# amazon-science/instruct-video-to-video

Hardware: AMD Instinct MI355X
Metric: denoised video-frames/sec (16f@256x384, 50 DDIM steps) (higher is better)
Workload: dtype fp16; 1 GPU; C2: 1 clip/step = VAE-encode + 50 DDIM steps (3-way CFG, text 7.5 / video 1.5) + VAE-decode, 16 frames @ 256x384, random-init full-width UNet+VAE; 5 independent clips in flight per GPU (stacked into every UNet launch, B = 3 x clips); frames=16, height=256, width=384, ddim_steps=50, clips_per_gpu=5, parallelism=clip-parallel x1, one all_gather, hip_graph=True, cfg_branch_streams=False, concurrent_clips=5, clip_mode=stacked, driver_mode=False, full=False

## Files before the change

### instruct-video-to-video_amd/csrc/gemm.hip

```cpp
#include "common.h"
#include <algorithm>
#include "gemm_dma.h"
#include <type_traits>
#include <cstdlib>

typedef unsigned uint4r __attribute__((ext_vector_type(4)));

struct RowInfo {
    int base;
    int oh, ow;
    bool valid;
};

#ifdef INSV2V_GEMM_PROF
__device__ unsigned long long g_prof[8];
#define PROF_MARK(i) do { if (tid == 0) prof_t[i] = wall_clock64(); } while (0)
#else
#define PROF_MARK(i) do { } while (0)
#endif

template <int W>
__device__ __forceinline__ float lane_group_sum(float v) {
    static_assert(W == 4 || W == 8 || W == 16, "a DPP row is 16 lanes");
    auto dpp = [](float x, auto ctrl) {
// ... 910 lines not shown
        if (b11 >= 200 || nk < 64) return 1;
        s = (int)(512 / b11);
        if (s > nk / 16) s = nk / 16;
        if (s > 8) s = 8;
    }
    if (s < 2) return 1;
    if ((int64_t)s * d.M * d.N * 4 > d.workspace_bytes) return 1;
    return s;
}

static int stats_tile_width(const insv2v_gemm_desc& d) {
    if (d.mode != INSV2V_MODE_LINEAR || d.c_fp32 || d.act == INSV2V_ACT_GEGLU || d.batch > 1 || (d.N & 7) || (d.ldc & 7) ||
        ((uintptr_t)d.c & 15) || (d.residual && ((d.ldr & 7) || ((uintptr_t)d.residual & 15) || (int64_t)d.M * d.ldr * 2 >= ((int64_t)1 << 31))))
        return 0;
    int shape = d.tile % 10;
    if (d.tile >= 240 && d.tile <= 249) return (d.N % 320 || d.k_split) ? 0 : 160;
    if (d.tile >= 100) return 0;
    if (d.tile == 0) {
        insv2v_gemm_desc dd = d;
        if (!dd.stats_out) dd.stats_out = (float*)(uintptr_t)16;
        if (dd.batch <= 0) dd.batch = 1;
        if (pick_pingpong(dd) == 2) return 160;
    }
    if (shape == 0) shape = pick_tile(d);
    switch (shape) {
        case 1: case 2: case 5: case 6: case 8: return 128;
        case 3: case 4: case 7: case 9: return 64;
    }
    return 0;
}

static int64_t g_operand_window = 0;
extern "C" int64_t insv2v_set_operand_window(int64_t bytes) {
    const int64_t prev = g_operand_window;
    g_operand_window = bytes > 0 ? bytes : 0;
    return prev;
}
static int64_t operand_window() { return g_operand_window > 0 ? g_operand_window : ((int64_t)1 << 31) - ((int64_t)1 << 20); }
static bool beyond_window(const insv2v_gemm_desc& d) {
    const bool conv = d.mode == INSV2V_MODE_CONV3X3;
    const int64_t a_rows = conv ? (int64_t)d.NB * d.IH * d.IW : (int64_t)d.M;
    const int64_t esz = d.c_fp32 ? 4 : 2;
    const int64_t big_in = std::max(a_rows * d.lda * 2, d.k_split ? a_rows * d.lda2 * 2 : (int64_t)0);
    const int64_t big_out = std::max((int64_t)d.M * d.ldc * esz, d.residual ? (int64_t)d.M * d.ldr * 2 : (int64_t)0);
    return big_in >= operand_window() || big_out >= operand_window();
}

extern "C" int insv2v_gemm_stats_parts(const insv2v_gemm_desc* dp) {
    if (!dp) return 0;
    insv2v_gemm_desc d = *dp;
    if (d.batch <= 0) d.batch = 1;
    if (beyond_window(d)) return 0;
    const int w = stats_tile_width(d);
    return w ? (d.N + w - 1) / w : 0;
}

static insv2v_gemm_desc finished_stats_of(insv2v_gemm_desc dd, hipStream_t s) {
    if (dd.stats_parts > 0) {
        hipLaunchKernelGGL(ln_finalize_kernel, dim3((dd.M + 255) / 256), dim3(256), 0, s, (const float2*)dd.row_stats,
                           (float2*)dd.stats_scratch, dd.M, dd.stats_parts, dd.K, dd.ln_eps);
        dd.row_stats = dd.stats_scratch; dd.stats_parts = 0;
    }
    return dd;
}

extern "C" int insv2v_gemm(const insv2v_gemm_desc* dp, insv2v_stream_t stream) {
    if (!one_device()) return INSV2V_EINVAL;
    if (!dp) return INSV2V_EINVAL;
    insv2v_gemm_desc d = *dp;
    if (!d.a || !d.w || !d.c || d.M <= 0 || d.N <= 0 || d.K <= 0) return INSV2V_EINVAL;
    if ((d.K & 7) || (d.lda & 7) || (d.ldw & 7)) return INSV2V_EINVAL;
    if (((uintptr_t)d.a | (uintptr_t)d.w) & 15) return INSV2V_EINVAL;
    if (d.k_split) {
        if (!d.a2 || (d.k_split % BK) || (d.lda2 & 7) || ((uintptr_t)d.a2 & 15)) return INSV2V_EINVAL;
    }
    if (d.row_bias && d.rows_per_group <= 0) return INSV2V_EINVAL;
    if (d.row_stats && (!d.col_sum || d.batch > 1)) return INSV2V_EINVAL;
    if (d.stats_parts < 0 || (d.stats_parts > 0 && (!d.row_stats || !d.stats_scratch))) return INSV2V_EINVAL;
    if (d.stats_out && stats_tile_width(d) == 0) return INSV2V_EUNSUPPORTED;
    if (d.act == INSV2V_ACT_GEGLU && (d.N % 64)) return INSV2V_EINVAL;
    if (d.act < 0 || d.act > INSV2V_ACT_TANH) return INSV2V_EINVAL;
    if (d.batch <= 0) d.batch = 1;
    if (d.alpha == 0.f) d.alpha = 1.f;
    if (d.w_group_rows < 0 || (d.w_group_rows > 0 && (d.w_group_rows % 256 || d.w_group_stride <= 0))) return INSV2V_EINVAL;
    if (d.w_group_rows > 0) {
        if (d.mode != INSV2V_MODE_LINEAR || d.batch > 1 || d.c_fp32 || d.act != INSV2V_ACT_NONE || d.residual || d.row_bias || d.row_stats || d.stats_out ||
            d.k_split || d.split_k > 1 || d.K < 256 || (d.N % 256 && d.N % 320))
            return INSV2V_EUNSUPPORTED;
    }
    if (d.gn_ab && (d.mode != INSV2V_MODE_CONV3X3 || d.gn_images_per_sample <= 0 || d.upsample)) return INSV2V_EINVAL;
    if (d.mode == INSV2V_MODE_CONV3X3) {
        if (d.Cin <= 0 || (d.Cin % BK) || d.K != 9 * d.Cin) return INSV2V_EINVAL;
        if ((long)d.NB * d.OH * d.OW != d.M || d.stride < 1) return INSV2V_EINVAL;
        if (d.upsample && (d.stride != 1 || d.pad_t != 1 || d.pad_l != 1 || (d.OH != 2 * d.IH && d.OH != 2 * d.IH - 1) || (d.OW != 2 * d.IW && d.OW != 2 * d.IW - 1)))
            return INSV2V_EINVAL;
    } else if (d.mode != INSV2V_MODE_LINEAR) {
        return INSV2V_EUNSUPPORTED;
    }
    {
        const bool conv = d.mode == INSV2V_MODE_CONV3X3;
        const int64_t lim = operand_window();
        if ((int64_t)d.N * d.ldw * 2 >= ((int64_t)1 << 31)) return INSV2V_EUNSUPPORTED;
        const int64_t esz = d.c_fp32 ? 4 : 2;
        if (beyond_window(d)) {
            if (d.batch > 1 || d.stats_out || d.split_k > 1) return INSV2V_EUNSUPPORTED;
            insv2v_gemm_desc f = finished_stats_of(d, as_stream(stream));
            auto lcm = [](int64_t a, int64_t b) { int64_t x = a, y = b; while (y) { const int64_t t = x % y; x = y; y = t; } return a / x * b; };
            const int64_t opix = conv ? (int64_t)d.OH * d.OW : 1, ipix = conv ? (int64_t)d.IH * d.IW : 1;
            int64_t unit = conv ? 1 : 2;
            if (d.row_bias) {
                const int64_t grp = (int64_t)d.rows_per_group * (d.rb_mod > 0 ? d.rb_mod : 1);
                if (conv && grp % opix) return INSV2V_EUNSUPPORTED;
                unit = lcm(unit, conv ? grp / opix : grp);
            }
            if (conv && d.gn_ab) unit = lcm(unit, d.gn_images_per_sample);
            if (!conv && unit < 256) unit = lcm(unit, 256);
            if (f.w_group_rows > 0) unit = lcm(unit, f.w_group_rows);
            const int64_t total = conv ? d.NB : d.M;
            const int64_t in_row = std::max((int64_t)d.lda * 2, d.k_split ? (int64_t)d.lda2 * 2 : (int64_t)0) * ipix;
            const int64_t out_row = std::max((int64_t)d.ldc * esz, d.residual ? (int64_t)d.ldr * 2 : (int64_t)0) * opix;
            int64_t per = (lim - 1) / std::max(in_row, out_row) / unit * unit;
            if (per <= 0) return INSV2V_EUNSUPPORTED;
            const int64_t nparts = (total + per - 1) / per;
            per = ((total + nparts - 1) / nparts + unit - 1) / unit * unit;
            for (int64_t u0 = 0; u0 < total; u0 += per) {
                const int64_t nu = std::min(per, total - u0);
                insv2v_gemm_desc s = f;
                const int64_t r_in = u0 * ipix, r_out = u0 * opix;
                s.a = (const char*)f.a + r_in * f.lda * 2;
                if (f.k_split) s.a2 = (const char*)f.a2 + r_in * f.lda2 * 2;
                s.c = (char*)f.c + r_out * f.ldc * esz;
                if (f.residual) s.residual = (const char*)f.residual + r_out * f.ldr * 2;
                if (f.row_stats) s.row_stats = f.row_stats + r_out * 2;
                if (f.w_group_rows > 0) s.w = (const char*)f.w + (r_out / f.w_group_rows) * f.w_group_stride * 2;
                if (f.row_bias && f.rb_mod <= 0) s.row_bias = f.row_bias + (r_out / f.rows_per_group) * f.ld_rb;
                if (conv && f.gn_ab) s.gn_ab = f.gn_ab + (u0 / f.gn_images_per_sample) * (int64_t)f.Cin * 2;
                s.M = (int32_t)(nu * opix);
                if (conv) s.NB = (int32_t)nu;
                const int rc = insv2v_gemm(&s, stream);
                if (rc != 0) return rc;
            }
            return 0;
        }
    }
    if (d.w_group_rows > 0) {
        const int64_t groups = ((int64_t)d.M + d.w_group_rows - 1) / d.w_group_rows;
        if (groups * d.w_group_stride * 2 >= ((int64_t)1 << 31)) return INSV2V_EUNSUPPORTED;
        const int cus = num_cus_gemm();
        const long tm = (d.M + 255) / 256, q_tiles = tm * ((d.N + 255) / 256), r_tiles = tm * ((d.N + 319) / 320);
        const bool r_ok = d.N % 320 == 0, q_ok = d.N % 256 == 0;
        const double q_cost = (double)((q_tiles + cus - 1) / cus) * 256 * 1.03, r_cost = (double)((r_tiles + cus - 1) / cus) * 320;
        const bool use_r = d.tile / 10 == 24 ? true : d.tile / 10 == 23 ? false : (r_ok && (!q_ok || r_cost <= q_cost));
        if (use_r ? !r_ok : !q_ok) return INSV2V_EUNSUPPORTED;
        return use_r ? insv2v_gemm_r8(d, 0, as_stream(stream)) : insv2v_gemm_q8(d, 0, as_stream(stream));
    }
    auto finished_stats = [&](const insv2v_gemm_desc& dd) { return finished_stats_of(dd, as_stream(stream)); };
    if (d.tile >= 200 && d.tile <= 206) return INSV2V_EUNSUPPORTED;
    if (d.tile >= 230 && d.tile <= 239) {
        if (d.split_k > 1 || d.stats_out) return INSV2V_EUNSUPPORTED;
        d.split_k = 1;
        return insv2v_gemm_q8(finished_stats(d), d.tile - 230, as_stream(stream));
    }
    if (d.tile >= 240 && d.tile <= 249) {
        if (d.split_k > 1) return INSV2V_EUNSUPPORTED;
        d.split_k = 1;
        return insv2v_gemm_r8(finished_stats(d), d.tile - 240, as_stream(stream));
    }
    if (d.tile >= 210 && d.tile <= 221) {
        if (d.split_k > 1 || d.stats_out) return INSV2V_EUNSUPPORTED;
        d.split_k = 1;
        return insv2v_gemm_w4(finished_stats(d), d.tile - 210, as_stream(stream));
    }
    int shape = d.tile % 10, pipe = d.tile / 10;
    const int nsplit = d.stats_out ? 1 : pick_split(d);
    insv2v_gemm_desc full = d;
    if (nsplit > 1) {
        d.c = d.workspace; d.ldc = d.N; d.c_fp32 = 1; d.c_bs = 0;
        d.bias = nullptr; d.row_bias = nullptr; d.residual = nullptr; d.act = INSV2V_ACT_NONE; d.alpha = 1.f;
        d.row_stats = nullptr; d.col_sum = nullptr;
        d.split_k = nsplit;
        if (shape == 0) shape = 5;
    } else {
        d.split_k = 1;
    }
    if (nsplit <= 1 && d.tile == 0 && !d.gn_ab) {
        const int pp = pick_pingpong(d);
        if (pp) {
            const insv2v_gemm_desc dd = finished_stats(d);
            const int rc = pp == 2 ? insv2v_gemm_r8(dd, 0, as_stream(stream)) : insv2v_gemm_q8(dd, 0, as_stream(stream));
            if (rc != INSV2V_EUNSUPPORTED || d.stats_out) return rc;
        }
    }
    if (nsplit <= 1 && d.tile == 0 && !d.stats_out && d.act == INSV2V_ACT_GEGLU && d.mode == INSV2V_MODE_LINEAR && !d.k_split && !d.residual) {
        static const int r8_geglu = getenv("INSV2V_R8_GEGLU") ? atoi(getenv("INSV2V_R8_GEGLU")) : 1;
        const int cus = num_cus_gemm();
        if (r8_geglu && cus > 0 && d.N % 320 == 0 && d.M >= 8192 && d.K >= 640 && !d.c_fp32 && d.batch <= 1) {
            const long tm = (d.M + 255) / 256, q_tiles = tm * ((d.N + 255) / 256), r_tiles = tm * (d.N / 320);
            const double q_cost = (double)((q_tiles + cus - 1) / cus) * 256 * 1.03, r_cost = (double)((r_tiles + cus - 1) / cus) * 320;
            if (r_cost <= q_cost) {
                const int rc = insv2v_gemm_r8(finished_stats(d), 0, as_stream(stream));
                if (rc != INSV2V_EUNSUPPORTED) return rc;
            }
        }
    }
    if (nsplit <= 1 && d.tile == 0 && !d.stats_out) {
        const int pick = pick_persistent(d);
        if (pick) {
            const insv2v_gemm_desc dd = finished_stats(d);
            const int rc = pick == 1 ? insv2v_gemm_q8(dd, 0, as_stream(stream)) : insv2v_gemm_w4(dd, 0, as_stream(stream));
            if (rc != INSV2V_EUNSUPPORTED) return rc;
        }
    }
    if (nsplit <= 1 && (d.tile == 100 || d.tile == 0)) {
        const int tws = halo_tw_shift(d);
        if (d.tile == 100 && tws < 0) return INSV2V_EUNSUPPORTED;
        if (d.tile == 100 && d.act >= INSV2V_ACT_RELU) return INSV2V_EUNSUPPORTED;
        if (tws >= 0 && d.act < INSV2V_ACT_RELU && (d.tile == 100 || ((long)d.M / 128) * ((d.N + 127) / 128) >= 200))
            return d.gn_ab ? launch_halo<4, 2, 1, 2, 1, true>(d, tws, as_stream(stream)) : launch_halo<4, 2, 1, 2, 1>(d, tws, as_stream(stream));
    }
    if (d.gn_ab) return INSV2V_EUNSUPPORTED;
    if (nsplit <= 1 && d.tile == 0 && d.mode == INSV2V_MODE_CONV3X3 && d.batch == 1 && !d.c_fp32 && d.M >= 10240 && d.N >= 640 && d.K >= 5760) {
        static const int enabled = getenv("INSV2V_GEMM_PERSISTENT") ? atoi(getenv("INSV2V_GEMM_PERSISTENT")) : 1;
        if (enabled) {
            const int rc = insv2v_gemm_q8(d, 0, as_stream(stream));
            if (rc != INSV2V_EUNSUPPORTED) return rc;
        }
    }
    if (d.tile >= 101 && d.tile <= 103 && d.act >= INSV2V_ACT_RELU) return INSV2V_EUNSUPPORTED;
    if (nsplit <= 1 && d.tile == 103) {
        int tws = halo_tw_shift(d);
        if (tws < 0 || d.gn_ab) return INSV2V_EUNSUPPORTED;
        if (d.OH % 16 == 0 && d.OW % 16 == 0) tws = 4;
        else if (d.OH % 32 == 0 && d.OW % 8 == 0) tws = 3;
        else return INSV2V_EUNSUPPORTED;
        return launch_halo<8, 2, 1, 2, 1, false, 3>(d, tws, as_stream(stream));
    }
    if (nsplit <= 1 && d.tile == 102) {
        const int tws = halo_tw_shift(d);
        if (tws < 0 || d.gn_ab) return INSV2V_EUNSUPPORTED;
        return launch_halo<2, 2, 2, 2, 1>(d, tws, as_stream(stream));
    }
    if (nsplit <= 1 && d.tile == 101) {
        const int tws = halo_tw_shift(d);
        if (tws < 0) return INSV2V_EUNSUPPORTED;
        return launch_halo<2, 2, 2, 2, 2>(d, tws, as_stream(stream));
    }
    if (shape == 0) shape = pick_tile(d);
    if (d.act == INSV2V_ACT_GEGLU && (shape == 3 || shape == 4 || shape == 7 || shape == 9)) shape = 2;
    if (pipe == 0) pipe = 2;
    hipStream_t s = as_stream(stream);
    const bool conv = d.mode == INSV2V_MODE_CONV3X3;
    int rc = INSV2V_EINVAL;
    switch (pipe) {
        case 2: rc = conv ? dispatch_tile<INSV2V_MODE_CONV3X3, 2>(d, shape, s) : dispatch_tile<INSV2V_MODE_LINEAR, 2>(d, shape, s); break;
        case 3: rc = conv ? dispatch_tile<INSV2V_MODE_CONV3X3, 3>(d, shape, s) : dispatch_tile<INSV2V_MODE_LINEAR, 3>(d, shape, s); break;
        case 4: rc = conv ? dispatch_tile<INSV2V_MODE_CONV3X3, 4>(d, shape, s) : dispatch_tile<INSV2V_MODE_LINEAR, 4>(d, shape, s); break;
    }
    if (rc != 0 || nsplit <= 1) return rc;
    const int64_t nchunk = (int64_t)full.M * (full.N / 8);
    hipLaunchKernelGGL(splitk_reduce_kernel, dim3((unsigned)((nchunk + 255) / 256)), dim3(256), 0, s, full, (const float*)full.workspace, nsplit);
    return launch_status();
}

extern "C" int insv2v_conv3x3_fuses_groupnorm(const insv2v_gemm_desc* dp) {
    if (!dp || dp->mode != INSV2V_MODE_CONV3X3 || dp->upsample || dp->split_k > 1) return 0;
    insv2v_gemm_desc d = *dp;
    if (d.batch <= 0) d.batch = 1;
    if (d.tile != 0 && d.tile != 100) return 0;
    if (halo_tw_shift(d) < 0) return 0;
    if (d.tile == 0 && (pick_split(d) > 1 || ((long)d.M / 128) * ((d.N + 127) / 128) < 200)) return 0;
    return 1;
}

#ifdef INSV2V_GEMM_PROF
extern "C" int insv2v_prof_read(unsigned long long* out, int reset) {
    hipError_t e = hipMemcpyFromSymbol(out, HIP_SYMBOL(g_prof), sizeof(unsigned long long) * 8);
    if (e == hipSuccess && reset) {
        unsigned long long z[8] = {0, 0, 0, 0, 0, 0, 0, 0};
        e = hipMemcpyToSymbol(HIP_SYMBOL(g_prof), z, sizeof(z));
    }
    return (int)e;
}
#endif
```

### instruct-video-to-video_amd/csrc/gemm_r8.hip

```cpp
#include "common.h"
#include "gemm_dma.h"
#include <type_traits>
#include <cstdlib>

namespace {

constexpr int BM = 256, BN = 320;
constexpr int AH_B = 128 * 128;
constexpr int WB_B = 64 * 128;
constexpr int W_BASE = 4 * AH_B;
constexpr int RING_B = 4 * AH_B + 10 * WB_B;
constexpr int PK_BIAS = 0, PK_CS = 2048, PK_ST = 4096, PK_RB = 6144, PARK_B = 8192;
constexpr int LDS_B = RING_B + 2 * PARK_B;

#ifndef R8_MID_SPREAD
#define R8_MID_SPREAD 1
#endif
#define SB() __builtin_amdgcn_sched_barrier(0)
#define BARRIER() do { SB(); __builtin_amdgcn_s_barrier(); SB(); } while (0)

typedef unsigned uint4v __attribute__((ext_vector_type(4)));
typedef unsigned uint2v __attribute__((ext_vector_type(2)));
__device__ __forceinline__ unsigned pack_h2(float x, float y) {
    typedef float f2_t __attribute__((ext_vector_type(2)));
    const f2_t v = {x, y};
    return __builtin_bit_cast(unsigned, __builtin_convertvector(v, half2v));
}
__device__ __forceinline__ float h_lo(unsigned u) { return (float)__builtin_bit_cast(half2v, u)[0]; }
__device__ __forceinline__ float h_hi(unsigned u) { return (float)__builtin_bit_cast(half2v, u)[1]; }

template <int I> using ic = std::integral_constant<int, I>;

template <int MODE, bool HAS_RES, int DBG = 0, bool SPLIT = true, bool STATS = false, bool GEGLU = false, bool CIM = false>
__global__ __launch_bounds__(512) void gemm_r8_kernel(insv2v_gemm_desc p, int dephase) {
    extern __shared__ __attribute__((aligned(16))) char smem[];
    const int tid = threadIdx.x, lane = tid & 63;
    const int wid = __builtin_amdgcn_readfirstlane(tid >> 6);
    const int wm = wid >> 1, wn = wid & 1, grp = wid >> 2;
    const int G = (int)gridDim.x;
    constexpr bool LIN = MODE == INSV2V_MODE_LINEAR;

    const int tiles_n = (p.N + BN - 1) / BN, tiles_m = (p.M + BM - 1) / BM, ntiles = tiles_m * tiles_n;
    if (dephase > 0 && ntiles > G) {
        const int n0 = ntiles % G;
        if (n0 != 0 && (int)blockIdx.x >= n0) {
            const float tile_cycles = (float)(p.K / BK) * 3700.f + (HAS_RES ? 30000.f : 10000.f);
            const float frac = (float)((int)blockIdx.x - n0 + 1) / (float)(G - n0 + 1) * (float)dephase * 0.001f;
            const unsigned long long wait = (unsigned long long)(frac * tile_cycles);
            unsigned long long t0, t1;
            asm volatile("s_memtime %0\n\ts_waitcnt lgkmcnt(0)" : "=s"(t0)::"memory");
            do {
                __builtin_amdgcn_s_sleep(64);
                asm volatile("s_memtime %0\n\ts_waitcnt lgkmcnt(0)" : "=s"(t1)::"memory");
            } while (t1 - t0 < wait);
        }
    }
    auto tile_origin = [&](int v, int& bm0, int& bn0) {
        const int bid = xcd_remap(v, ntiles);
        constexpr int GROUP_M = 8;
        const int per_group = GROUP_M * tiles_n;
        const int gidx = bid / per_group, first_m = gidx * GROUP_M;
        const int gsz = min(GROUP_M, tiles_m - first_m), rin = bid - gidx * per_group;
        const int tn = rin / gsz, tm = first_m + rin - tn * gsz;
        bm0 = tm * BM; bn0 = tn * BN;
    };

    const srd_t rA = make_srd(p.a), rA2 = make_srd(p.a2 ? p.a2 : p.a), rW = make_srd(p.w);
    const bool ln = p.row_stats != nullptr;

    const int prow = wid * 8 + (lane >> 3);
    const int chunk8 = ((lane & 7) ^ ((prow >> 1) & 7)) * 8;
    unsigned aoff[4];
    unsigned amask[2] = {0, 0};
    unsigned woff;
    unsigned amax = 0;
    const unsigned wmax = (unsigned)(((int64_t)(p.N - 1) * p.ldw + chunk8) * 2);
    const int nk = p.K / BK;
    const int IHu = p.upsample ? p.OH : p.IH, IWu = p.upsample ? p.OW : p.IW;
    const int ups = p.upsample ? 1 : 0;
    struct Cursor { int v, kt, k0, kh, kw, ci0, soffA, abm0; bool second; int tap, dpix; unsigned wbase; } cur = {(int)blockIdx.x, 0, 0, 0, 0, 0, 0, 0, false, 0, 0, 0u};
    if (CIM) cur.dpix = -p.IW - 1;
    auto refresh_aoff = [&]() {
        const int ld = (int)((SPLIT && cur.second) ? p.lda2 : p.lda);
        if (LIN) {
            aoff[0] = ((unsigned)(cur.abm0 + prow) * (unsigned)ld + (unsigned)chunk8) * 2u;
            amax = ((unsigned)(p.M - 1) * (unsigned)ld + (unsigned)chunk8) * 2u;
        } else {
            const float rOW = 1.0f / (float)p.OW, rOH = 1.0f / (float)p.OH;
#pragma unroll
            for (int r = 0; r < 4; ++r) {
                const int m = cur.abm0 + (r >> 1) * 128 + (r & 1) * 64 + prow;
                const bool okm = m < p.M;
                const int mm = okm ? m : 0;
                int t = (int)((float)mm * rOW);
                int ow = mm - t * p.OW;
                if (ow < 0) { ow += p.OW; --t; } else if (ow >= p.OW) { ow -= p.OW; ++t; }
                int nb = (int)((float)t * rOH);
                int oh = t - nb * p.OH;
                if (oh < 0) { oh += p.OH; --nb; } else if (oh >= p.OH) { oh -= p.OH; ++nb; }
                if (CIM) {
                    aoff[r] = (unsigned)(nb * p.IH * p.IW + oh * p.IW + ow);
                    const unsigned vh = (okm && oh > 0 ? 1u : 0u) | (okm ? 2u : 0u) | (okm && oh + 1 < p.IH ? 4u : 0u);
                    const unsigned vw = (ow > 0 ? 1u : 0u) | 2u | (ow + 1 < p.IW ? 4u : 0u);
                    const unsigned bits = ((vh & 1u) ? vw : 0u) | ((vh & 2u) ? vw << 3 : 0u) | ((vh & 4u) ? vw << 6 : 0u);
                    if (r & 1) amask[r >> 1] |= bits << 9; else amask[r >> 1] = bits;
                } else {
                    const int ih = oh * p.stride - p.pad_t + cur.kh, iw = ow * p.stride - p.pad_l + cur.kw;
                    const bool ok = okm && (unsigned)ih < (unsigned)IHu && (unsigned)iw < (unsigned)IWu;
                    const int pix = nb * p.IH * p.IW + (ih >> ups) * p.IW + (iw >> ups);
                    aoff[r] = ok ? (unsigned)((pix * ld + chunk8) * 2) : OOB_OFFSET;
                }
            }
        }
    };
    auto set_stage_rows = [&](int v) {
        int bm0 = 0, bn0 = 0;
        const bool live = v < ntiles;
        if (live) tile_origin(v, bm0, bn0);
        else { bm0 = p.M + BM; bn0 = p.N + BN; }
        cur.abm0 = bm0;
        cur.wbase = (LIN && live && p.w_group_rows > 0) ? (unsigned)((int64_t)(bm0 / p.w_group_rows) * p.w_group_stride * 2) : 0u;
        const int c32 = (wid & 3) * 8 + (lane >> 3);
        const int pc = ((c32 >> 2) & 3) * 8 + (c32 >> 4) * 4 + (c32 & 3);
        const int n = GEGLU ? bn0 + (c32 >> 4) * 32 + (c32 & 15) : bn0 + (wid >> 2) * 160 + pc;
        woff = ((unsigned)n * (unsigned)p.ldw + (unsigned)chunk8) * 2u;
    };
    auto advance = [&]() {
        bool newtile = false, refresh = false;
        if (++cur.kt == nk) {
            cur.v += G; cur.kt = 0; cur.k0 = 0; cur.kh = cur.kw = cur.ci0 = 0; cur.soffA = 0; cur.second = false;
            if (CIM) { cur.tap = 0; cur.dpix = -p.IW - 1; }
            newtile = true;
        } else if (CIM) {
            if (++cur.tap == 9) { cur.tap = 0; cur.ci0 += BK; }
            const int kh = (cur.tap * 11) >> 5, kw = cur.tap - 3 * kh;
            cur.dpix = (kh - 1) * p.IW + kw - 1;
            cur.second = SPLIT && p.k_split > 0 && cur.ci0 >= p.k_split;
            cur.soffA = (cur.ci0 - (cur.second ? p.k_split : 0)) * 2;
            cur.k0 = cur.tap * p.Cin + cur.ci0;
        } else {
            cur.k0 += BK; cur.soffA += BK * 2;
            if (LIN) {
                if (SPLIT && p.k_split > 0 && cur.k0 == p.k_split) { cur.second = true; cur.soffA = 0; refresh = true; }
            } else {
                cur.ci0 += BK;
                if (cur.ci0 >= p.Cin) {
                    cur.ci0 = 0; cur.soffA = 0;
                    if (++cur.kw == 3) { cur.kw = 0; ++cur.kh; }
                    cur.second = false; refresh = true;
                } else if (SPLIT && p.k_split > 0 && cur.ci0 == p.k_split) {
                    cur.second = true; cur.soffA = 0; refresh = true;
                }
            }
        }
        if (newtile) set_stage_rows(cur.v);
        if (newtile || refresh) refresh_aoff();
    };
    auto stage_a = [&](auto h_c, auto buf_c, int i) {
        constexpr int H = decltype(h_c)::value, BUF = decltype(buf_c)::value;
        char* dst = smem + (H * 2 + BUF) * AH_B + i * 8192 + wid * 1024;
        if (LIN) {
            const int ld = (int)((SPLIT && cur.second) ? p.lda2 : p.lda);
            dma16((SPLIT && cur.second) ? rA2 : rA, min(aoff[0] + (unsigned)((H * 128 + i * 64) * ld * 2), amax), cur.soffA, dst);
        } else if (CIM) {
            constexpr int R = H * 2;
            const unsigned ld2 = (unsigned)((SPLIT && cur.second) ? p.lda2 : p.lda) * 2u;
            const bool ok = (amask[H] >> (i * 9 + cur.tap)) & 1u;
            const unsigned off = __umul24(aoff[R + i] + (unsigned)cur.dpix, ld2) + (unsigned)(chunk8 * 2);
            dma16((SPLIT && cur.second) ? rA2 : rA, ok ? off : OOB_OFFSET, cur.soffA, dst);
        } else {
            dma16((SPLIT && cur.second) ? rA2 : rA, aoff[H * 2 + i], cur.soffA, dst);
        }
    };
    auto stage_w = [&](auto pb_c, auto buf_c) {
        constexpr int PB = decltype(pb_c)::value, BUF = decltype(buf_c)::value;
        char* dst = smem + W_BASE + (PB * 2 + BUF) * WB_B + wid * 1024;
        if (GEGLU) {
            const int t = (wid >> 2) * 5 + PB;
            dma16(rW, min(woff + (unsigned)(((t >> 1) * 64 + (t & 1) * 16) * (int)p.ldw * 2), wmax), cur.k0 * 2 + (int)cur.wbase, dst);
        } else {
            dma16(rW, min(woff + (unsigned)(PB * 32 * (int)p.ldw * 2), wmax), cur.k0 * 2 + (int)cur.wbase, dst);
        }
    };
    auto row_group = [&](int m) { int g = m / p.rows_per_group; if (p.rb_mod > 0) g %= p.rb_mod; return g; };
    auto stage_park = [&](int pb, int bm0, int bn0) {
        char* park = smem + RING_B + pb * PARK_B;
        const srd_t rBias = make_srd(p.bias ? (const void*)p.bias : p.w), rCs = make_srd(ln ? (const void*)p.col_sum : p.w),
// ... 103 lines not shown
    const unsigned lds0 = (unsigned)(uintptr_t)(__attribute__((address_space(3))) char*)smem;
    auto park6 = [&](unsigned a, floatx4& b0, floatx4& b1, floatx4& r0, floatx4& r1, floatx4& c0, floatx4& c1) {
        if constexpr (GEGLU)
            asm volatile("ds_read_b128 %0, %6\n\tds_read_b128 %1, %6 offset:128\n\tds_read_b128 %2, %6 offset:6144\n\t"
                         "ds_read_b128 %3, %6 offset:6272\n\tds_read_b128 %4, %6 offset:2048\n\tds_read_b128 %5, %6 offset:2176\n\t"
                         "s_waitcnt lgkmcnt(0)"
                         : "=&v"(b0), "=&v"(b1), "=&v"(r0), "=&v"(r1), "=&v"(c0), "=&v"(c1) : "v"(a) : "memory");
        else
            asm volatile("ds_read_b128 %0, %6\n\tds_read_b128 %1, %6 offset:16\n\tds_read_b128 %2, %6 offset:6144\n\t"
                         "ds_read_b128 %3, %6 offset:6160\n\tds_read_b128 %4, %6 offset:2048\n\tds_read_b128 %5, %6 offset:2064\n\t"
                         "s_waitcnt lgkmcnt(0)"
                         : "=&v"(b0), "=&v"(b1), "=&v"(r0), "=&v"(r1), "=&v"(c0), "=&v"(c1) : "v"(a) : "memory");
    };
    auto stat4 = [&](unsigned a, float2& s0, float2& s1, float2& s2, float2& s3) {
        asm volatile("ds_read_b64 %0, %4\n\tds_read_b64 %1, %4 offset:128\n\tds_read_b64 %2, %4 offset:256\n\tds_read_b64 %3, %4 offset:384\n\t"
                     "s_waitcnt lgkmcnt(0)" : "=&v"(s0), "=&v"(s1), "=&v"(s2), "=&v"(s3) : "v"(a) : "memory");
    };
    auto epilogue = [&](int bm0, int bn0, int pb) {
        if (DBG == 2 || DBG == 5) {
            float s = 0.f;
#pragma unroll
            for (int i = 0; i < 5; ++i)
#pragma unroll
                for (int tb = 0; tb < 4; ++tb)
#pragma unroll
                    for (int cb = 0; cb < 2; ++cb)
#pragma unroll
                        for (int r = 0; r < 4; ++r) s += acc[i][tb][cb][r];
            if (s == 12345.678f) ((half_t*)p.c)[tid] = (half_t)s;
            return;
        }
        unsigned elane;
        asm volatile("v_mbcnt_lo_u32_b32 %0, -1, 0\n\tv_mbcnt_hi_u32_b32 %0, -1, %0" : "=v"(elane));
        const int e15 = (int)(elane & 15), eg = (int)(elane >> 4);
        const srd_t rC = make_srd(p.c), rR = make_srd(p.residual ? p.residual : p.c);
        const unsigned park = lds0 + RING_B + pb * PARK_B;
        float ra[LIN ? 4 : 1], rm[LIN ? 4 : 1];
        unsigned offc[4], offr[4];
        {
            float2 st[4];
            if (LIN) stat4(park + PK_ST + (wm * 64 + e15) * 8, st[0], st[1], st[2], st[3]);
            else { ra[0] = p.alpha; rm[0] = 0.f; }
#pragma unroll
            for (int tb = 0; tb < 4; ++tb) {
                const int m = bm0 + wm * 64 + tb * 16 + e15;
                if (LIN) {
                    const float mean = ln ? st[tb].x : 0.f, rstd = ln ? st[tb].y : 1.f;
                    ra[tb] = rstd * p.alpha; rm[tb] = -rstd * mean;
                }
                offc[tb] = m < p.M ? (unsigned)(m * (int)p.ldc * 2 + eg * (GEGLU ? 8 : 16)) : OOB_OFFSET;
                offr[tb] = m < p.M ? (unsigned)(m * (int)p.ldr * 2 + eg * 16) : OOB_OFFSET;
            }
        }
        if constexpr (GEGLU) {
#pragma unroll
            for (int pbk = 0; pbk < 5; ++pbk) {
                const int t = wn * 5 + pbk;
                const int nl = (t >> 1) * 64 + (t & 1) * 16 + 4 * eg;
                float bh[4], ch[4], bg[4], cg[4];
                {
                    floatx4 tb_[2], tr[2], tc[2];
                    park6(park + nl * 4, tb_[0], tb_[1], tr[0], tr[1], tc[0], tc[1]);
#pragma unroll
                    for (int e = 0; e < 4; ++e) { bh[e] = tb_[0][e] + tr[0][e]; ch[e] = tc[0][e]; bg[e] = tb_[1][e] + tr[1][e]; cg[e] = tc[1][e]; }
                }
                const int on = (bn0 >> 1) + t * 16;
                const bool okc = on + eg * 4 + 4 <= (p.N >> 1);
#pragma unroll
                for (int tb = 0; tb < 4; ++tb) {
                    float v[4];
#pragma unroll
                    for (int e = 0; e < 4; ++e) {
                        const float x = fmaf(ra[LIN ? tb : 0], acc[pbk][tb][0][e], fmaf(rm[LIN ? tb : 0], ch[e], bh[e]));
                        const float g = fmaf(ra[LIN ? tb : 0], acc[pbk][tb][1][e], fmaf(rm[LIN ? tb : 0], cg[e], bg[e]));
                        v[e] = x * gelu_erf_f(g);
                    }
                    const uint2v out = {pack_h2(v[0], v[1]), pack_h2(v[2], v[3])};
                    __builtin_amdgcn_raw_buffer_store_b64(out, rC, okc ? offc[tb] : OOB_OFFSET, on * 2, 0);
                    asm volatile("s_nop 7" ::"v"(out));
                }
            }
            return;
        }
        uint4v rv[2][4];
        auto load_res = [&](auto pbk_c, auto slot_c) {
            constexpr int PBK = decltype(pbk_c)::value, SLOT = decltype(slot_c)::value;
            const int on = bn0 + wn * 160 + PBK * 32;
            const bool okc = on + eg * 8 + 8 <= p.N;
#pragma unroll
            for (int tb = 0; tb < 4; ++tb) rv[SLOT][tb] = __builtin_amdgcn_raw_buffer_load_b128(rR, okc ? offr[tb] : OOB_OFFSET, on * 2, 0);
        };
        if (HAS_RES) {
            load_res(ic<0>{}, ic<0>{}); load_res(ic<1>{}, ic<1>{});
            asm volatile("s_waitcnt vmcnt(0)" ::: "memory");
            SB();
        }
        float st1[4] = {0.f, 0.f, 0.f, 0.f}, st2[4] = {0.f, 0.f, 0.f, 0.f};
#pragma unroll
        for (int pbk = 0; pbk < 5; ++pbk) {
            const int slot = pbk & 1;
            if (HAS_RES && (pbk == 2 || pbk == 4)) { asm volatile("s_waitcnt vmcnt(0)" ::: "memory"); SB(); }
            const int cl = wn * 160 + pbk * 32 + 8 * eg;
            float bs[8], cs[8];
            {
                floatx4 tb_[2], tr[2], tc[2];
                park6(park + cl * 4, tb_[0], tb_[1], tr[0], tr[1], tc[0], tc[1]);
#pragma unroll
                for (int h = 0; h < 2; ++h)
#pragma unroll
                    for (int e = 0; e < 4; ++e) { bs[4 * h + e] = tb_[h][e] + tr[h][e]; cs[4 * h + e] = tc[h][e]; }
            }
            const int on = bn0 + wn * 160 + pbk * 32;
            const bool okc = on + eg * 8 + 8 <= p.N;
#pragma unroll
            for (int tb = 0; tb < 4; ++tb) {
                float v[8];
#pragma unroll
                for (int h = 0; h < 2; ++h)
#pragma unroll
                    for (int e = 0; e < 4; ++e) v[4 * h + e] = fmaf(ra[LIN ? tb : 0], acc[pbk][tb][h][e], fmaf(rm[LIN ? tb : 0], cs[4 * h + e], bs[4 * h + e]));
                if (HAS_RES) {
                    const uint4v r = rv[slot][tb];
                    v[0] += h_lo(r[0]); v[1] += h_hi(r[0]); v[2] += h_lo(r[1]); v[3] += h_hi(r[1]);
                    v[4] += h_lo(r[2]); v[5] += h_hi(r[2]); v[6] += h_lo(r[3]); v[7] += h_hi(r[3]);
                }
                if (STATS) {
#pragma unroll
                    for (int e = 0; e < 8; ++e) { st1[tb] += v[e]; st2[tb] = fmaf(v[e], v[e], st2[tb]); }
                }
                const uint4v out = {pack_h2(v[0], v[1]), pack_h2(v[2], v[3]), pack_h2(v[4], v[5]), pack_h2(v[6], v[7])};
                __builtin_amdgcn_raw_buffer_store_b128(out, rC, okc ? offc[tb] : OOB_OFFSET, on * 2, 0);
                asm volatile("s_nop 7" ::"v"(out));
            }
            if (HAS_RES) {
                SB();
                if (pbk == 0) load_res(ic<2>{}, ic<0>{});
                if (pbk == 1) load_res(ic<3>{}, ic<1>{});
                if (pbk == 2) load_res(ic<4>{}, ic<0>{});
                SB();
            }
        }
        if (STATS) {
            const int part = bn0 / 160 + wn;
#pragma unroll
            for (int tb = 0; tb < 4; ++tb) {
                const int m = bm0 + wm * 64 + tb * 16 + e15;
                float s1 = st1[tb] + __shfl_xor(st1[tb], 16, 64), s2 = st2[tb] + __shfl_xor(st2[tb], 16, 64);
                s1 += __shfl_xor(s1, 32, 64); s2 += __shfl_xor(s2, 32, 64);
                if (eg == 0 && m < p.M) *(float2*)(p.stats_out + ((int64_t)part * p.M + m) * 2) = make_float2(s1, s2);
            }
        }
    };

    int cbm0, cbn0;
    int cv = blockIdx.x, cpb = 0;
    tile_origin(cv, cbm0, cbn0);
    set_stage_rows(cv);
    refresh_aoff();
    stage_park(0, cbm0, cbn0);
    stage_a(ic<0>{}, ic<0>{}, 0); stage_a(ic<0>{}, ic<0>{}, 1); stage_a(ic<1>{}, ic<0>{}, 0); stage_a(ic<1>{}, ic<0>{}, 1);
    stage_w(ic<0>{}, ic<0>{}); stage_w(ic<1>{}, ic<0>{}); stage_w(ic<2>{}, ic<0>{}); stage_w(ic<3>{}, ic<0>{}); stage_w(ic<4>{}, ic<0>{});
    advance();
    stage_a(ic<0>{}, ic<1>{}, 0); stage_a(ic<0>{}, ic<1>{}, 1); stage_a(ic<1>{}, ic<1>{}, 0); stage_a(ic<1>{}, ic<1>{}, 1);
    stage_w(ic<0>{}, ic<1>{}); stage_w(ic<1>{}, ic<1>{});
    wait_vmcnt<6>();
    BARRIER();
    zero_acc();

    auto tile_step = [&](auto buf_c, bool first, int nbm0, int nbn0, int npb) {
        constexpr int B = decltype(buf_c)::value;
        read_w(ic<B>{}, ic<0>{});
        SB();
        read_a(ic<B>{});
        SB();
        if (first) stage_park(npb, nbm0, nbn0);
        BARRIER();
        mma(ic<0>{}, [&](int i) { if (i == 0) stage_w(ic<2>{}, ic<B ^ 1>{}); else stage_w(ic<3>{}, ic<B ^ 1>{}); });
        BARRIER();
        read_w(ic<B>{}, ic<1>{});
        BARRIER();
        mma(ic<1>{}, [&](int i) { if (i == 0) stage_w(ic<4>{}, ic<B ^ 1>{}); });
        BARRIER();
        read_w(ic<B>{}, ic<2>{});
        advance();
        BARRIER();
        mma(ic<2>{}, [&](int i) { stage_a(ic<0>{}, ic<B>{}, i); });
        BARRIER();
        read_w(ic<B>{}, ic<3>{});
        BARRIER();
        mma(ic<3>{}, [&](int i) { stage_a(ic<1>{}, ic<B>{}, i); });
        BARRIER();
        read_w(ic<B>{}, ic<4>{});
        wait_vmcnt<4>();
        BARRIER();
        mma(ic<4>{}, [&](int i) { if (i == 0) stage_w(ic<0>{}, ic<B>{}); else stage_w(ic<1>{}, ic<B>{}); });
        BARRIER();
    };
    int par = 0;
    unsigned long long cyc_loop = 0, cyc_join = 0, cyc_epi = 0, ntl = 0, ts0 = 0, ts1 = 0, ts2 = 0, ts3 = 0;
    auto stamp = [&](unsigned long long& t) { if (DBG == 4) asm volatile("s_memtime %0\n\ts_waitcnt lgkmcnt(0)" : "=s"(t)::"memory"); };
    for (; cv < ntiles; cv += G) {
        tile_origin(cv, cbm0, cbn0);
        stamp(ts0);
        if (grp == 1) BARRIER();
        bool first = cv != (int)blockIdx.x;
        int t = 0;
        if (par) { tile_step(ic<1>{}, first, cbm0, cbn0, cpb); first = false; t = 1; par = 0; }
        for (; t + 1 < nk; t += 2) {
            tile_step(ic<0>{}, first, cbm0, cbn0, cpb);
            first = false;
            tile_step(ic<1>{}, false, cbm0, cbn0, cpb);
        }
        if (t < nk) { tile_step(ic<0>{}, first, cbm0, cbn0, cpb); par = 1; }
        stamp(ts1);
        if (grp == 0) BARRIER();
        stamp(ts2);
        epilogue(cbm0, cbn0, cpb);
        stamp(ts3);
        if (DBG == 4) { cyc_loop += ts1 - ts0; cyc_join += ts2 - ts1; cyc_epi += ts3 - ts2; ++ntl; }
        zero_acc();
        cpb ^= 1;
    }
    if (DBG == 5 && p.workspace && blockIdx.x < 64 && lane == 0) {
        unsigned* o = (unsigned*)p.workspace + ((int)blockIdx.x * 8 + wid) * 12;
#pragma unroll
        for (int i = 0; i < 5; ++i) { o[i] = dbg_seg[i]; o[5 + i] = dbg_gap[i]; }
        o[10] = dbg_n; o[11] = 0;
    }
    if (DBG == 4 && p.workspace && blockIdx.x < 64 && lane == 0) {
        unsigned long long* o = (unsigned long long*)p.workspace + ((int)blockIdx.x * 8 + wid) * 4;
        o[0] = cyc_loop; o[1] = cyc_join; o[2] = cyc_epi; o[3] = ntl;
    }
}

template <int MODE, bool HAS_RES, int DBG = 0, bool SPLIT = true, bool STATS = false, bool GEGLU = false, bool CIM = false>
int launch_r8(const insv2v_gemm_desc& d, hipStream_t s) {
    static bool attr_set = false;
    static int num_cu = 0;
    if (!attr_set) {
        hipError_t e = hipFuncSetAttribute((const void*)gemm_r8_kernel<MODE, HAS_RES, DBG, SPLIT, STATS, GEGLU, CIM>, hipFuncAttributeMaxDynamicSharedMemorySize, LDS_B);
        if (e != hipSuccess) return (int)e;
        int dev = 0;
        hipDeviceProp_t prop;
        if (hipGetDevice(&dev) != hipSuccess || hipGetDeviceProperties(&prop, dev) != hipSuccess) return INSV2V_EINVAL;
        num_cu = prop.multiProcessorCount;
        attr_set = true;
    }
    const int tiles = ((d.M + BM - 1) / BM) * ((d.N + BN - 1) / BN);
    static const int dephase = getenv("INSV2V_R8_DEPHASE") ? atoi(getenv("INSV2V_R8_DEPHASE")) : 0;
    hipLaunchKernelGGL((gemm_r8_kernel<MODE, HAS_RES, DBG, SPLIT, STATS, GEGLU, CIM>), dim3(tiles < num_cu ? tiles : num_cu), dim3(512), LDS_B, s, d, dephase);
    return launch_status();
}

}

int insv2v_gemm_r8(const insv2v_gemm_desc& d, int variant, hipStream_t s) {
    if (d.batch > 1 || d.c_fp32 || d.split_k > 1) return INSV2V_EUNSUPPORTED;
    if ((d.K % BK) || (d.N & 7) || (d.ldc & 7) || ((uintptr_t)d.c & 15)) return INSV2V_EUNSUPPORTED;
    if (d.residual && ((d.ldr & 7) || ((uintptr_t)d.residual & 15))) return INSV2V_EUNSUPPORTED;
    if (d.k_split && (d.k_split % BK)) return INSV2V_EUNSUPPORTED;
    const bool geglu = d.act == INSV2V_ACT_GEGLU;
    if (d.act != INSV2V_ACT_NONE && !geglu) return INSV2V_EUNSUPPORTED;
    if (geglu && (d.mode != INSV2V_MODE_LINEAR || (d.N % BN) || d.residual || d.k_split > 0 || d.stats_out || variant != 0)) return INSV2V_EUNSUPPORTED;
    if (d.row_stats && (d.M & 1)) return INSV2V_EUNSUPPORTED;
    if (d.row_bias && ((d.ld_rb & 3) || (d.rows_per_group % 256 && d.M > d.rows_per_group))) return INSV2V_EUNSUPPORTED;
    if ((int64_t)d.M * d.ldc * 2 >= ((int64_t)1 << 31) || (d.residual && (int64_t)d.M * d.ldr * 2 >= ((int64_t)1 << 31))) return INSV2V_EUNSUPPORTED;
    if ((d.bias && ((uintptr_t)d.bias & 15)) || (d.col_sum && ((uintptr_t)d.col_sum & 15)) || (d.row_bias && ((uintptr_t)d.row_bias & 15)))
        return INSV2V_EUNSUPPORTED;
    const bool conv = d.mode == INSV2V_MODE_CONV3X3;
    if (conv && ((d.Cin % BK) || d.M >= (1 << 24))) return INSV2V_EUNSUPPORTED;
    const bool res = d.residual != nullptr;
    constexpr int L = INSV2V_MODE_LINEAR, C = INSV2V_MODE_CONV3X3;
    if (geglu) return launch_r8<L, false, 0, false, false, true>(d, s);
    if (d.stats_out) {
        if (conv || d.k_split > 0 || (d.N % BN) || variant != 0) return INSV2V_EUNSUPPORTED;
        return res ? launch_r8<L, true, 0, false, true>(d, s) : launch_r8<L, false, 0, false, true>(d, s);
    }
    static const bool cim_on = !(getenv("INSV2V_R8_CIM") && atoi(getenv("INSV2V_R8_CIM")) == 0);
    const bool cim = conv && cim_on && d.stride == 1 && !d.upsample && d.pad_t == 1 && d.pad_l == 1 && d.IH == d.OH && d.IW == d.OW;
    if (cim && (variant == 0 || variant == 4)) {
        if (variant == 4) return res ? launch_r8<C, true, 4, true, false, false, true>(d, s) : launch_r8<C, false, 4, true, false, false, true>(d, s);
        if (d.k_split > 0) return res ? launch_r8<C, true, 0, true, false, false, true>(d, s) : launch_r8<C, false, 0, true, false, false, true>(d, s);
        return res ? launch_r8<C, true, 0, false, false, false, true>(d, s) : launch_r8<C, false, 0, false, false, false, true>(d, s);
    }
    switch (variant) {
        case 0:
            if (d.k_split > 0) {
                if (conv) return res ? launch_r8<C, true>(d, s) : launch_r8<C, false>(d, s);
                return res ? launch_r8<L, true>(d, s) : launch_r8<L, false>(d, s);
            }
            if (conv) return res ? launch_r8<C, true, 0, false>(d, s) : launch_r8<C, false, 0, false>(d, s);
            return res ? launch_r8<L, true, 0, false>(d, s) : launch_r8<L, false, 0, false>(d, s);
        case 2:
            if (conv) return launch_r8<C, false, 2>(d, s);
            return launch_r8<L, false, 2>(d, s);
        case 5:
            if (conv) return launch_r8<C, false, 5>(d, s);
            return launch_r8<L, false, 5>(d, s);
        case 4:
            if (conv) return res ? launch_r8<C, true, 4>(d, s) : launch_r8<C, false, 4>(d, s);
            return res ? launch_r8<L, true, 4>(d, s) : launch_r8<L, false, 4>(d, s);
    }
    return INSV2V_EINVAL;
}
```

Before: 16.27 frames/s.

## Overlap r8 GEMM epilogue with next tile's main loop via rolling epilogue

Adds a ROLL template mode to the persistent r8 GEMM kernel. The previous tile's output is written in fragments interleaved between the MMA phases of the next tile, instead of in a separate epilogue after the loop. It also adds a LayerNorm-folded variant for LINEAR problems with row stats. The aim is to hide epilogue store and convert latency behind compute. The cost is more register pressure and more complex scheduling. For non-residual problems with K >= 2*BK this becomes the default variant-0 path.

```diff
diff --git a/instruct-video-to-video_amd/csrc/gemm.hip b/instruct-video-to-video_amd/csrc/gemm.hip
--- a/instruct-video-to-video_amd/csrc/gemm.hip
+++ b/instruct-video-to-video_amd/csrc/gemm.hip
@@ -1086,7 +1086,7 @@
         const double q_cost = (double)((q_tiles + cus - 1) / cus) * 256 * 1.03, r_cost = (double)((r_tiles + cus - 1) / cus) * 320;
         const bool use_r = d.tile / 10 == 24 ? true : d.tile / 10 == 23 ? false : (r_ok && (!q_ok || r_cost <= q_cost));
         if (use_r ? !r_ok : !q_ok) return INSV2V_EUNSUPPORTED;
-        return use_r ? insv2v_gemm_r8(d, 0, as_stream(stream)) : insv2v_gemm_q8(d, 0, as_stream(stream));
+        return use_r ? insv2v_gemm_r8(d, d.tile / 10 == 24 ? d.tile - 240 : 0, as_stream(stream)) : insv2v_gemm_q8(d, 0, as_stream(stream));
     }
     auto finished_stats = [&](const insv2v_gemm_desc& dd) { return finished_stats_of(dd, as_stream(stream)); };
     if (d.tile >= 200 && d.tile <= 206) return INSV2V_EUNSUPPORTED;
diff --git a/instruct-video-to-video_amd/csrc/gemm_r8.hip b/instruct-video-to-video_amd/csrc/gemm_r8.hip
--- a/instruct-video-to-video_amd/csrc/gemm_r8.hip
+++ b/instruct-video-to-video_amd/csrc/gemm_r8.hip
@@ -31,8 +31,10 @@
 
 template <int I> using ic = std::integral_constant<int, I>;
 
-template <int MODE, bool HAS_RES, int DBG = 0, bool SPLIT = true, bool STATS = false, bool GEGLU = false, bool CIM = false>
+template <int MODE, bool HAS_RES, int DBG = 0, bool SPLIT = true, bool STATS = false, bool GEGLU = false, bool CIM = false, int ROLL = 0>
 __global__ __launch_bounds__(512) void gemm_r8_kernel(insv2v_gemm_desc p, int dephase) {
+    static_assert(ROLL == 0 || (!HAS_RES && !STATS && !GEGLU && DBG != 2), "the rolling epilogue exists for the plain forms only");
+    static_assert(ROLL != 2 || MODE == INSV2V_MODE_LINEAR, "only a LINEAR problem carries a folded LayerNorm");
     extern __shared__ __attribute__((aligned(16))) char smem[];
     const int tid = threadIdx.x, lane = tid & 63;
     const int wid = __builtin_amdgcn_readfirstlane(tid >> 6);
@@ -442,6 +444,67 @@
         }
     };
 
+    unsigned long long cyc_loop = 0, cyc_join = 0, cyc_epi = 0, ntl = 0, ts0 = 0, ts1 = 0, ts2 = 0, ts3 = 0;
+    auto stamp = [&](unsigned long long& t) { if (DBG == 4) asm volatile("s_memtime %0\n\ts_waitcnt lgkmcnt(0)" : "=s"(t)::"memory"); };
+    auto epi_frag = [&](auto pbk_c, int bm0, int bn0, int pb) {
+        constexpr int PBK = decltype(pbk_c)::value;
+        constexpr bool LNF = ROLL == 2;
+        stamp(ts2);
+        unsigned elane;
+        asm volatile("v_mbcnt_lo_u32_b32 %0, -1, 0\n\tv_mbcnt_hi_u32_b32 %0, -1, %0" : "=v"(elane));
+        const int e15 = (int)(elane & 15), eg = (int)(elane >> 4);
+        const srd_t rC = make_srd(p.c);
+        const unsigned park = lds0 + RING_B + pb * PARK_B;
+        const int on = bn0 + wn * 160 + PBK * 32;
+        const bool okc = on + eg * 8 + 8 <= p.N;
+        float ra[LNF ? 4 : 1], rm[LNF ? 4 : 1];
+        if constexpr (LNF) {
+            float2 st[4];
+            stat4(park + PK_ST + (wm * 64 + e15) * 8, st[0], st[1], st[2], st[3]);
+#pragma unroll
+            for (int tb = 0; tb < 4; ++tb) { ra[tb] = st[tb].y * p.alpha; rm[tb] = -st[tb].y * st[tb].x; }
+        } else { ra[0] = p.alpha; rm[0] = 0.f; }
+        uint2v out[4][2];
+#pragma unroll
+        for (int h = 0; h < 2; ++h) {
+            floatx4 tb_, tr, tc;
+            float bs[4], cs[4];
+            const unsigned pa = park + (wn * 160 + PBK * 32 + 8 * eg + 4 * h) * 4;
+            if constexpr (LNF)
+                asm volatile("ds_read_b128 %0, %3\n\tds_read_b128 %1, %3 offset:6144\n\tds_read_b128 %2, %3 offset:2048\n\ts_waitcnt lgkmcnt(0)"
+                             : "=&v"(tb_), "=&v"(tr), "=&v"(tc) : "v"(pa) : "memory");
+            else
+                asm volatile("ds_read_b128 %0, %2\n\tds_read_b128 %1, %2 offset:6144\n\ts_waitcnt lgkmcnt(0)" : "=&v"(tb_), "=&v"(tr) : "v"(pa) : "memory");
+#pragma unroll
+            for (int e = 0; e < 4; ++e) {
+                bs[e] = LIN ? tb_[e] + tr[e] : (tb_[e] + tr[e]) + 0.f;
+                if constexpr (LNF) cs[e] = tc[e];
+            }
+#pragma unroll
+            for (int tb = 0; tb < 4; ++tb) {
+                float v[4];
+#pragma unroll
+                for (int e = 0; e < 4; ++e) {
+                    if constexpr (LNF) v[e] = fmaf(ra[tb], acc[PBK][tb][h][e], fmaf(rm[tb], cs[e], bs[e]));
+                    else v[e] = fmaf(ra[0], acc[PBK][tb][h][e], bs[e]);
+                }
+                out[tb][h] = uint2v{pack_h2(v[0], v[1]), pack_h2(v[2], v[3])};
+            }
+        }
+#pragma unroll
+        for (int tb = 0; tb < 4; ++tb) {
+            const int m = bm0 + wm * 64 + tb * 16 + e15;
+            const unsigned offc = (m < p.M && okc) ? (unsigned)(m * (int)p.ldc * 2 + eg * 16) : OOB_OFFSET;
+            const uint4v o = {out[tb][0][0], out[tb][0][1], out[tb][1][0], out[tb][1][1]};
+            __builtin_amdgcn_raw_buffer_store_b128(o, rC, offc, on * 2, 0);
+            asm volatile("s_nop 7" ::"v"(o));
+            acc[PBK][tb][0] = floatx4{0.f, 0.f, 0.f, 0.f}; acc[PBK][tb][1] = floatx4{0.f, 0.f, 0.f, 0.f};
+        }
+        stamp(ts3);
+        if (DBG == 4) cyc_epi += ts3 - ts2;
+    };
+    constexpr bool EPI_FRONT = ROLL != 0 && !(LIN && ROLL == 1);
+
     int cbm0, cbn0;
     int cv = blockIdx.x, cpb = 0;
     tile_origin(cv, cbm0, cbn0);
@@ -457,38 +520,66 @@
     BARRIER();
     zero_acc();
 
-    auto tile_step = [&](auto buf_c, bool first, int nbm0, int nbn0, int npb) {
+    auto tile_step = [&](auto buf_c, bool first, int nbm0, int nbn0, int npb, bool last = false, int obm0 = 0, int obn0 = 0) {
         constexpr int B = decltype(buf_c)::value;
+        if constexpr (EPI_FRONT) { if (first) epi_frag(ic<4>{}, obm0, obn0, npb ^ 1); SB(); }
         read_w(ic<B>{}, ic<0>{});
         SB();
         read_a(ic<B>{});
         SB();
         if (first) stage_park(npb, nbm0, nbn0);
+        if constexpr (ROLL != 0 && !EPI_FRONT) { SB(); if (first) epi_frag(ic<4>{}, obm0, obn0, npb ^ 1); }
         BARRIER();
         mma(ic<0>{}, [&](int i) { if (i == 0) stage_w(ic<2>{}, ic<B ^ 1>{}); else stage_w(ic<3>{}, ic<B ^ 1>{}); });
         BARRIER();
+        if constexpr (EPI_FRONT) { if (last) epi_frag(ic<0>{}, nbm0, nbn0, npb); SB(); }
         read_w(ic<B>{}, ic<1>{});
+        if constexpr (ROLL != 0 && !EPI_FRONT) { SB(); if (last) epi_frag(ic<0>{}, nbm0, nbn0, npb); }
         BARRIER();
         mma(ic<1>{}, [&](int i) { if (i == 0) stage_w(ic<4>{}, ic<B ^ 1>{}); });
         BARRIER();
+        if constexpr (EPI_FRONT) { if (last) epi_frag(ic<1>{}, nbm0, nbn0, npb); SB(); }
         read_w(ic<B>{}, ic<2>{});
         advance();
+        if constexpr (ROLL != 0 && !EPI_FRONT) { SB(); if (last) epi_frag(ic<1>{}, nbm0, nbn0, npb); }
         BARRIER();
         mma(ic<2>{}, [&](int i) { stage_a(ic<0>{}, ic<B>{}, i); });
         BARRIER();
+        if constexpr (EPI_FRONT) { if (last) epi_frag(ic<2>{}, nbm0, nbn0, npb); SB(); }
         read_w(ic<B>{}, ic<3>{});
+        if constexpr (ROLL != 0 && !EPI_FRONT) { SB(); if (last) epi_frag(ic<2>{}, nbm0, nbn0, npb); }
         BARRIER();
         mma(ic<3>{}, [&](int i) { stage_a(ic<1>{}, ic<B>{}, i); });
         BARRIER();
+        if constexpr (EPI_FRONT) { if (last) { wait_vmcnt<4>(); epi_frag(ic<3>{}, nbm0, nbn0, npb); } SB(); }
         read_w(ic<B>{}, ic<4>{});
-        wait_vmcnt<4>();
+        if (!(EPI_FRONT && last)) wait_vmcnt<4>();
+        if constexpr (ROLL != 0 && !EPI_FRONT) { SB(); if (last) epi_frag(ic<3>{}, nbm0, nbn0, npb); }
         BARRIER();
         mma(ic<4>{}, [&](int i) { if (i == 0) stage_w(ic<0>{}, ic<B>{}); else stage_w(ic<1>{}, ic<B>{}); });
         BARRIER();
     };
     int par = 0;
-    unsigned long long cyc_loop = 0, cyc_join = 0, cyc_epi = 0, ntl = 0, ts0 = 0, ts1 = 0, ts2 = 0, ts3 = 0;
-    auto stamp = [&](unsigned long long& t) { if (DBG == 4) asm volatile("s_memtime %0\n\ts_waitcnt lgkmcnt(0)" : "=s"(t)::"memory"); };
+    if constexpr (ROLL != 0) {
+        if (grp == 1) BARRIER();
+        int obm0 = 0, obn0 = 0;
+        bool prev = false;
+        for (; cv < ntiles; cv += G) {
+            tile_origin(cv, cbm0, cbn0);
+            stamp(ts0);
+            auto step = [&](auto buf_c, int t) { tile_step(buf_c, t == 0 && prev, cbm0, cbn0, cpb, t == nk - 1, obm0, obn0); };
+            int t = 0;
+            if (par) { step(ic<1>{}, 0); t = 1; par = 0; }
+            for (; t + 1 < nk; t += 2) { step(ic<0>{}, t); step(ic<1>{}, t + 1); }
+            if (t < nk) { step(ic<0>{}, t); par = 1; }
+            stamp(ts1);
+            if (DBG == 4) { cyc_loop += ts1 - ts0; ++ntl; }
+            obm0 = cbm0; obn0 = cbn0; prev = true;
+            cpb ^= 1;
+        }
+        if (prev) epi_frag(ic<4>{}, obm0, obn0, cpb ^ 1);
+        if (grp == 0) BARRIER();
+    } else
     for (; cv < ntiles; cv += G) {
         tile_origin(cv, cbm0, cbn0);
         stamp(ts0);
@@ -523,12 +614,12 @@
     }
 }
 
-template <int MODE, bool HAS_RES, int DBG = 0, bool SPLIT = true, bool STATS = false, bool GEGLU = false, bool CIM = false>
+template <int MODE, bool HAS_RES, int DBG = 0, bool SPLIT = true, bool STATS = false, bool GEGLU = false, bool CIM = false, int ROLL = 0>
 int launch_r8(const insv2v_gemm_desc& d, hipStream_t s) {
     static bool attr_set = false;
     static int num_cu = 0;
     if (!attr_set) {
-        hipError_t e = hipFuncSetAttribute((const void*)gemm_r8_kernel<MODE, HAS_RES, DBG, SPLIT, STATS, GEGLU, CIM>, hipFuncAttributeMaxDynamicSharedMemorySize, LDS_B);
+        hipError_t e = hipFuncSetAttribute((const void*)gemm_r8_kernel<MODE, HAS_RES, DBG, SPLIT, STATS, GEGLU, CIM, ROLL>, hipFuncAttributeMaxDynamicSharedMemorySize, LDS_B);
         if (e != hipSuccess) return (int)e;
         int dev = 0;
         hipDeviceProp_t prop;
@@ -538,20 +629,21 @@
     }
     const int tiles = ((d.M + BM - 1) / BM) * ((d.N + BN - 1) / BN);
     static const int dephase = getenv("INSV2V_R8_DEPHASE") ? atoi(getenv("INSV2V_R8_DEPHASE")) : 0;
-    hipLaunchKernelGGL((gemm_r8_kernel<MODE, HAS_RES, DBG, SPLIT, STATS, GEGLU, CIM>), dim3(tiles < num_cu ? tiles : num_cu), dim3(512), LDS_B, s, d, dephase);
+    hipLaunchKernelGGL((gemm_r8_kernel<MODE, HAS_RES, DBG, SPLIT, STATS, GEGLU, CIM, ROLL>), dim3(tiles < num_cu ? tiles : num_cu), dim3(512), LDS_B, s, d, dephase);
     return launch_status();
 }
 
 }
 
 int insv2v_gemm_r8(const insv2v_gemm_desc& d, int variant, hipStream_t s) {
+    if (variant == 3 || variant < 0 || variant > 6) return INSV2V_EINVAL;
     if (d.batch > 1 || d.c_fp32 || d.split_k > 1) return INSV2V_EUNSUPPORTED;
     if ((d.K % BK) || (d.N & 7) || (d.ldc & 7) || ((uintptr_t)d.c & 15)) return INSV2V_EUNSUPPORTED;
     if (d.residual && ((d.ldr & 7) || ((uintptr_t)d.residual & 15))) return INSV2V_EUNSUPPORTED;
     if (d.k_split && (d.k_split % BK)) return INSV2V_EUNSUPPORTED;
     const bool geglu = d.act == INSV2V_ACT_GEGLU;
     if (d.act != INSV2V_ACT_NONE && !geglu) return INSV2V_EUNSUPPORTED;
-    if (geglu && (d.mode != INSV2V_MODE_LINEAR || (d.N % BN) || d.residual || d.k_split > 0 || d.stats_out || variant != 0)) return INSV2V_EUNSUPPORTED;
+    if (geglu && (d.mode != INSV2V_MODE_LINEAR || (d.N % BN) || d.residual || d.k_split > 0 || d.stats_out || variant > 1)) return INSV2V_EUNSUPPORTED;
     if (d.row_stats && (d.M & 1)) return INSV2V_EUNSUPPORTED;
     if (d.row_bias && ((d.ld_rb & 3) || (d.rows_per_group % 256 && d.M > d.rows_per_group))) return INSV2V_EUNSUPPORTED;
     if ((int64_t)d.M * d.ldc * 2 >= ((int64_t)1 << 31) || (d.residual && (int64_t)d.M * d.ldr * 2 >= ((int64_t)1 << 31))) return INSV2V_EUNSUPPORTED;
@@ -563,11 +655,31 @@
     constexpr int L = INSV2V_MODE_LINEAR, C = INSV2V_MODE_CONV3X3;
     if (geglu) return launch_r8<L, false, 0, false, false, true>(d, s);
     if (d.stats_out) {
-        if (conv || d.k_split > 0 || (d.N % BN) || variant != 0) return INSV2V_EUNSUPPORTED;
+        if (conv || d.k_split > 0 || (d.N % BN) || variant > 1) return INSV2V_EUNSUPPORTED;
         return res ? launch_r8<L, true, 0, false, true>(d, s) : launch_r8<L, false, 0, false, true>(d, s);
     }
     static const bool cim_on = !(getenv("INSV2V_R8_CIM") && atoi(getenv("INSV2V_R8_CIM")) == 0);
     const bool cim = conv && cim_on && d.stride == 1 && !d.upsample && d.pad_t == 1 && d.pad_l == 1 && d.IH == d.OH && d.IW == d.OW;
+    const bool roll = !res && d.K >= 2 * BK && !(cim && d.k_split > 0) && !(conv && d.row_stats);
+    if (roll && (variant == 0 || variant == 4 || variant == 6)) {
+        const bool lnf = d.row_stats != nullptr;
+        if (variant == 6) {
+            if (cim) return launch_r8<C, false, 5, false, false, false, true, 1>(d, s);
+            if (conv) return launch_r8<C, false, 5, true, false, false, false, 1>(d, s);
+            return lnf ? launch_r8<L, false, 5, true, false, false, false, 2>(d, s) : launch_r8<L, false, 5, true, false, false, false, 1>(d, s);
+        }
+        if (variant == 4) {
+            if (cim) return launch_r8<C, false, 4, false, false, false, true, 1>(d, s);
+            if (conv) return launch_r8<C, false, 4, true, false, false, false, 1>(d, s);
+            return lnf ? launch_r8<L, false, 4, true, false, false, false, 2>(d, s) : launch_r8<L, false, 4, true, false, false, false, 1>(d, s);
+        }
+        if (cim) return launch_r8<C, false, 0, false, false, false, true, 1>(d, s);
+        if (conv) return d.k_split > 0 ? launch_r8<C, false, 0, true, false, false, false, 1>(d, s) : launch_r8<C, false, 0, false, false, false, false, 1>(d, s);
+        if (lnf) return d.k_split > 0 ? launch_r8<L, false, 0, true, false, false, false, 2>(d, s) : launch_r8<L, false, 0, false, false, false, false, 2>(d, s);
+        return d.k_split > 0 ? launch_r8<L, false, 0, true, false, false, false, 1>(d, s) : launch_r8<L, false, 0, false, false, false, false, 1>(d, s);
+    }
+    if (variant == 6) return INSV2V_EUNSUPPORTED;
+    if (variant == 1) variant = 0;
     if (cim && (variant == 0 || variant == 4)) {
         if (variant == 4) return res ? launch_r8<C, true, 4, true, false, false, true>(d, s) : launch_r8<C, false, 4, true, false, false, true>(d, s);
         if (d.k_split > 0) return res ? launch_r8<C, true, 0, true, false, false, true>(d, s) : launch_r8<C, false, 0, true, false, false, true>(d, s);
```

After: 16.19 frames/s. Within noise of the previous version (-0.5%).
